# SensorsINI/v2e

Hardware: AMD Instinct MI355X
Metric: Mevents/s (EventEmulator.generate_events, 346x260, 10x slowdown) (higher is better)
Workload: dtype f64

## Files before the change

### v2e_amd/csrc/emu.hip

```cpp
#include "common.h"
#include "../../include/v2e_detmath.h"

#include <cstdarg>
#include <cstdlib>
#include <chrono>
#include <vector>

namespace {

constexpr int BLOCK = 256;
constexpr int WAVE = 64;
constexpr int RING = 64;
constexpr int SCAN_BLOCKS = 64;
constexpr int STAMP_LAUNCHES = 128;

constexpr uint32_t CNT_MASK = 0x00FFFFFFu;
constexpr uint32_t CNT_NEG = 1u << 24;
constexpr uint32_t CNT_SHOT_ON = 1u << 25;
constexpr uint32_t CNT_SHOT_OFF = 1u << 26;

struct FrameCtl {
    double t_prev, t_frame;
    double dt_over_tau;
    double shot_base;
// ... 579 lines not shown
                const unsigned long long row = ev0 + it_base + cidx;
                if (row < cap) ev[row] = make_float4(t, fx, fy, neg ? -1.0f : 1.0f);
                else dropped = true;
                ++fcount;
            }
        }
        carry += chunk_total;
    }
    const uint32_t son_tot = trow[2 * M], soff_tot = trow[2 * M + 1];
    if (a.do_shot) {
        const bool s_on = (cw & CNT_SHOT_ON) != 0, s_off = (cw & CNT_SHOT_OFF) != 0;
        const unsigned long long so = __ballot(s_on), sf = __ballot(s_off);
        if (so | sf) {
            const float tl = tg(n - 1);
            if (s_on) {
                const unsigned long long row = ev0 + carry + hrow[(size_t)(2 * M) * a.nwaves + w] + (uint32_t)__popcll(so & lt);
                if (row < cap) ev[row] = make_float4(tl, fx, fy, 1.0f);
                else dropped = true;
            }
            if (s_off) {
                const unsigned long long row = ev0 + carry + son_tot + hrow[(size_t)(2 * M + 1) * a.nwaves + w] + (uint32_t)__popcll(sf & lt);
                if (row < cap) ev[row] = make_float4(tl, fx, fy, -1.0f);
                else dropped = true;
            }
        }
    }
    if (valid) {
        const bool shot = a.do_shot && (cw & (CNT_SHOT_ON | CNT_SHOT_OFF));
        if (fcount > 0 || shot) {
            R b = ((R *)a.base)[sp];
            const float dp = (float)(neg ? 0 : fcount) * a.pos_thres[sp];
            const float dn = (float)(neg ? fcount : 0) * a.neg_thres[sp];
            b = b + (R)dp;
            b = b - (R)dn;
            if (shot) b = ((R *)a.lp)[sp];
            ((R *)a.base)[sp] = b;
        }
        if (use_refr && fcount > 0) a.ts_mem[sp] = tsm;
    }
    if (__ballot(dropped) != 0ull && lane == 0) atomicOr(&rec[clip].flags, V2E_FLAG_EVENTS_DROPPED);
    if (w == 0 && lane == 0) {
        rec[clip].n_signal = carry;
        rec[clip].n_events = carry + (a.do_shot ? son_tot + soff_tot : 0u);
        rec[clip].n_on = sum_on + (a.do_shot ? son_tot : 0u);
        rec[clip].n_off = sum_off + (a.do_shot ? soff_tot : 0u);
        rec[clip].ev_offset = ev0;
    }
}

__global__ __launch_bounds__(BLOCK) void k_permute(const float4 *__restrict__ in, float4 *__restrict__ out,
                                                   const int32_t *__restrict__ idx, unsigned long long row0,
                                                   unsigned long long n)
{
    const unsigned long long j = (unsigned long long)blockIdx.x * BLOCK + threadIdx.x;
    if (j < n) out[row0 + j] = in[row0 + (unsigned long long)idx[j]];
}

struct FrameScratch {
    v2e_frame_rec rec[2];
    FrameCtl ctl;
};

__global__ __launch_bounds__(256) void k_frame_rows_to_host(const float4 *__restrict__ ev, const v2e_frame_rec *__restrict__ rec,
                                                            float4 *__restrict__ out_rows, v2e_frame_rec *__restrict__ out_rec,
                                                            unsigned long long row0, unsigned long long max_rows,
                                                            v2e_frame_rec *__restrict__ rec_next)
{
    const v2e_frame_rec r = *rec;
    if (blockIdx.x == 0 && threadIdx.x == 0) {
        if (out_rec) *out_rec = r;
        if (rec_next) {
            v2e_frame_rec z;
            memset(&z, 0, sizeof(z));
            *rec_next = z;
        }
    }
    if (r.flags & (V2E_FLAG_EVENTS_DROPPED | V2E_FLAG_ITERS_CLAMPED)) return;
    const unsigned long long n = r.n_events < row0 + max_rows ? r.n_events : row0 + max_rows;
    for (unsigned long long i = row0 + (unsigned long long)blockIdx.x * 256 + threadIdx.x; i < n; i += (unsigned long long)gridDim.x * 256)
        out_rows[i] = ev[i];
}

#include "emu_chain.h"

}

namespace {
__global__ void k_zero_words(uint32_t *p, size_t n)
{
    const size_t i = (size_t)blockIdx.x * 256 + threadIdx.x;
    if (i < n) p[i] = 0u;
}
struct ZeroRanges { uint32_t *p[4]; unsigned long long n[4]; };
__global__ __launch_bounds__(256) void k_zero_ranges(ZeroRanges z)
{
    const unsigned long long i = (unsigned long long)blockIdx.x * 256 + threadIdx.x;
    unsigned long long base = 0;
#pragma unroll
    for (int r = 0; r < 4; ++r) {
        if (i >= base && i < base + z.n[r]) z.p[r][i - base] = 0u;
        base += z.n[r];
    }
}
}
static inline hipError_t zero_async(void *p, size_t bytes, hipStream_t s)
{
    const size_t n = (bytes + 3) / 4;
    if (n == 0) return hipSuccess;
    k_zero_words<<<(unsigned)((n + 255) / 256), 256, 0, s>>>((uint32_t *)p, n);
    return hipGetLastError();
}

struct RunScratch {
    FrameCtl *run_ctl = nullptr;
    uint32_t *run_fidx = nullptr;
    const void **run_frames = nullptr;
    unsigned long long **stamp_slot = nullptr;
    unsigned long long *run_off = nullptr;
    uint32_t *ch_gM = nullptr;
    unsigned *ch_bar = nullptr;
    uint2 *ch_rec = nullptr;
    uint32_t *ch_cnt = nullptr;
    uint32_t *ch_ruleM = nullptr;
    float *ch_tsold = nullptr;
    uint16_t *ch_wmax = nullptr;
    uint16_t *ch_wtot = nullptr;
    CFrame *ch_cf = nullptr;
    unsigned *ch_cdone = nullptr;
    uint32_t *ch_cT = nullptr, *ch_ckbase = nullptr, *ch_cperm = nullptr, *ch_cpre = nullptr;
    uint32_t *ch_cmask = nullptr;
    uint32_t *ch_cpre16 = nullptr;
    void free_chain()
    {
        auto drop = [](auto *&b) { hipFree((void *)b); b = nullptr; };
        drop(ch_gM); drop(ch_bar); drop(ch_rec); drop(ch_cnt); drop(ch_ruleM); drop(ch_tsold); drop(ch_wmax); drop(ch_wtot);
        drop(ch_cf); drop(ch_cdone); drop(ch_cT); drop(ch_ckbase); drop(ch_cperm); drop(ch_cpre); drop(ch_cmask); drop(ch_cpre16);
    }
    void free_all()
    {
        free_chain();
        auto drop = [](auto *&b) { hipFree((void *)b); b = nullptr; };
        drop(run_ctl); drop(run_fidx); drop(run_frames); drop(stamp_slot); drop(run_off);
    }
};

struct v2e_emu {
    int H, W, n_clips, max_iters, device;
    int npx, nwaves, nkeys_cap;
    long long npx_pad;
    void *lp = nullptr, *base = nullptr;
    float *ts_mem = nullptr, *pos_thres = nullptr, *neg_thres = nullptr, *noise_rate = nullptr;
    uint32_t *cnt = nullptr, *hist = nullptr, *tot = nullptr;
    void *pn_arr = nullptr;
    const float *pn_tape = nullptr;
    void *sc_hp = nullptr, *sc_prev = nullptr;
    const void *cs_sur = nullptr;
    void *csr_scratch = nullptr, *csr_lp = nullptr;
    std::vector<double> csr_ap, csr_ah;
    std::vector<int> csr_steps;
    double csr_thr = 0.0;
    int *csr_steps_dev = nullptr;
    unsigned long long *csr_slots = nullptr;
    int csr_slots_cap = 0;
    float *sc_tau = nullptr;
    uint32_t sc_first_frame = 0;
    double *dbg_lognew = nullptr, *dbg_cms = nullptr, *dbg_diff = nullptr;
// ... 1013 lines not shown
            V2E_HIP(hipDeviceSynchronize());
        }
        if (n_launch > h->ch_launch_cap) {
            h->sync_runs();
            for (RunScratch &q : h->sets) { hipFree(q.ch_gM); hipFree(q.ch_bar); q.ch_gM = nullptr; q.ch_bar = nullptr; }
            h->ch_launch_cap = n_launch;
            h->drop_graphs();
        }
        if (!r.ch_gM) {
            V2E_HIP(hipMalloc(&r.ch_gM, sizeof(uint32_t) * (size_t)h->ch_launch_cap * (K + 1) * h->n_clips * K));
            V2E_HIP(hipMalloc(&r.ch_bar, sizeof(unsigned) * (size_t)h->ch_launch_cap * 2 * K * h->n_clips));
            h->drop_graphs();
        }
    }
    return 0;
}

static bool chain_eligible(const v2e_emu *h, const v2e_emu_params *p, int dtype)
{
    if (h->max_iters > CHAIN_MAX_ITERS) return false;
    if (dtype == V2E_DT_F64 && p->log_input) return false;
    if (p->photoreceptor_noise) return false;
    if (h->sc_hp) return false;
    if (h->cs_sur) return false;
    return true;
}

enum class ChainMode {
    plain,
    captured,
    pipelined,
    profiled,
};
struct ChainMarks { std::vector<hipEvent_t> chain, rows; };

static int enqueue_run_chain(v2e_emu *h, const v2e_emu_params *p, const KArgs &a_in, int dtype, int n_frames, float *events,
                             uint64_t cap, v2e_frame_rec *recs, hipStream_t s, ChainMode mode, ChainMarks *marks = nullptr)
{
    const bool captured = mode == ChainMode::captured, pipelined = mode == ChainMode::pipelined;
    const RunScratch &r = h->cur();
    const size_t esz = dtype == V2E_DT_U8 ? 1 : (dtype == V2E_DT_F32 ? 4 : 8);
    const bool has_refr = p->refractory_period_s > 0;
    const int K = h->ch_K, E = h->ch_E, m = E / K, D = h->ch_D, NC = h->n_clips, nD = h->ch_nD;
    const bool fused_rec = h->ch_fused != 0;
    const std::vector<ChainLaunch> plan = chain_plan(n_frames, K, E, nD, has_refr, fused_rec);
    const int nL = (int)plan.size();
    const int nB = (n_frames + K - 1) / K;
    const int nEB = (n_frames + E - 1) / E;
    KArgs a = a_in;
    Sched sc;
    sc.h = h; sc.st[ST_MAIN] = s; sc.st[ST_AHEAD] = h->ahead; sc.st[ST_SIDE] = h->side; sc.st[ST_TAB] = h->tabs; sc.st[ST_SIDE2] = h->side2;
    if (mode == ChainMode::profiled)
        for (int q = 0; q < ST_COUNT; ++q) sc.st[q] = s;
    auto mark = [&](bool rows, hipStream_t stq) -> int {
        if (mode != ChainMode::profiled) return 0;
        hipEvent_t e;
        V2E_HIP(hipEventCreate(&e));
        (rows ? marks->rows : marks->chain).push_back(e);
        V2E_HIP(hipEventRecord(e, stq));
        return 0;
    };
    int gy = NC;
    if (has_refr && K > 1) gy = std::max(1, std::min(NC, h->ch_max_blocks / std::max(h->ngroups, 1)));
    dim3 grid(h->ngroups, gy);
    const int tab_stream = captured || pipelined ? ST_SIDE : ST_TAB;
    constexpr int NSET = 3;
    auto launch_emission = [&](int b, int ef0, int enE) -> int {
        CEmitArgs ea;
        memset(&ea, 0, sizeof(ea));
        ea.ctl = r.run_ctl; ea.recs = recs; ea.fidx_base = r.run_fidx;
        ea.f0 = ef0; ea.nE = enE; ea.D = D; ea.n_clips = NC; ea.slot0 = ef0 % D;
        ea.nwp = h->ch_nwp; ea.nwaves = chain_egroups(h); ea.E = E;
        ea.cnt = r.ch_cnt; ea.tsold = has_refr ? r.ch_tsold : nullptr; ea.ruleM = has_refr ? r.ch_ruleM : nullptr;
        const size_t set = (size_t)(b % NSET) * E * NC;
        ea.wmax = r.ch_wmax + set * h->ch_nwp; ea.wtot = r.ch_wtot + set * h->nkeys_cap * h->ch_nwp;
        ea.cf = r.ch_cf + set; ea.cT = r.ch_cT + set * h->nkeys_cap; ea.ckbase = r.ch_ckbase + set * h->nkeys_cap;
        ea.cperm = r.ch_cperm + set * h->max_iters * 8; ea.cpre = r.ch_cpre + set * h->nkeys_cap * h->ch_nwp;
        ea.cdone = r.ch_cdone + set;
        const bool pull = r.ch_cmask != nullptr;
        ea.cmask = pull ? r.ch_cmask + set * h->ch_nwp * h->nkeys_cap * 2 * GPX : nullptr;
        bool two = h->ch_nwp > 1024;
        if (const char *ev = getenv("V2E_AMD_PULL_TWO_LEVEL")) two = atoi(ev) != 0;
        ea.cpre16 = pull && two ? r.ch_cpre16 + set * h->nkeys_cap * (h->ch_nwp / 16) : nullptr;
        ea.wpf = std::max(4, std::min(two ? 128 : 64, h->npx / 2048));
        ea.p2 = two ? 16 : 64;
        while (ea.p2 < (two ? h->ch_nwp / 16 : ea.nwaves)) ea.p2 *= 2;
        ea.events = (float4 *)events; ea.cap = cap;
        ea.off_in = r.run_off + (size_t)b * NC;
        ea.off_out = r.run_off + (size_t)(b + 1) * NC;
        ea.ich = 4;
        ea.capw = GROUP_PX * ea.ich;
        ea.coff_in_cemit = captured || pipelined ? 1 : 0;
        ea.zpw_tot = CTOT_ZF;
        ea.zpw_emit = 1;
        const int REC_LDS = (ea.capw + WAVE) * 4 * (BLOCK / WAVE);
        const int egx = (chain_egroups(h) + BLOCK / WAVE - 1) / (BLOCK / WAVE);
        void *args[] = {(void *)&a, (void *)&ea};
        if (sc.wait(tab_stream, EV_FORK, b)) return V2E_EHIP;
        if (b >= NSET && !captured && sc.wait(tab_stream, EV_JOIN, b - NSET)) return V2E_EHIP;
        if (sc.kernel(tab_stream, (const void *)k_ctot, dim3(egx, NC, (ea.nE + CTOT_ZF - 1) / CTOT_ZF), dim3(BLOCK), 0, args)) return V2E_EHIP;
        if (h->ch_nwp <= 4096) {
            if (sc.kernel(tab_stream, (const void *)k_cframe1, dim3(1, NC, ea.nE), dim3(CFRAME_THREADS), 0, args)) return V2E_EHIP;
        } else if (sc.kernel(tab_stream, (const void *)k_cframe, dim3(std::min(h->nkeys_cap, CFRAME_ROWS), NC, ea.nE), dim3(CFRAME_THREADS), 0, args)) {
            return V2E_EHIP;
        }
        const int row_stream = pipelined ? ST_SIDE2 : captured ? ST_SIDE : ((b & 1) ? ST_SIDE2 : ST_SIDE);
        if (!ea.coff_in_cemit) {
            void *oargs[] = {(void *)&ea};
            if (sc.kernel(tab_stream, (const void *)k_coff, dim3(NC), dim3(WAVE), 0, oargs)) return V2E_EHIP;
        }
        if (sc.record(EV_TAB, b, tab_stream)) return V2E_EHIP;
        if (!captured && sc.wait(row_stream, EV_TAB, b)) return V2E_EHIP;
        if (mark(true, sc.st[row_stream])) return V2E_EHIP;
        if (pull) {
            if (sc.kernel(row_stream, ea.cpre16 ? (const void *)k_cpull<true> : (const void *)k_cpull<false>, dim3(8 * ea.wpf * ((ea.nE + 7) / 8), NC), dim3(BLOCK), (size_t)(2 * ea.p2 * 4), args)) return V2E_EHIP;
        } else if (sc.kernel(row_stream, (const void *)k_cemit, dim3(egx, NC, ea.nE), dim3(BLOCK), (size_t)REC_LDS, args)) return V2E_EHIP;
        if (mark(true, sc.st[row_stream])) return V2E_EHIP;
        return sc.record(EV_JOIN, b, row_stream);
    };
    const bool split0 = m > 1 && n_frames > K && !pipelined;
    const bool ahead_whole = pipelined && !fused_rec && n_frames <= D;
    auto launch_ahead = [&](int b) -> int {
        if (!ahead_whole && b >= nD && sc.wait(ST_AHEAD, EV_CHAIN, (b - nD + 1) * m)) return V2E_EHIP;
        const int b0 = ahead_whole ? 0 : b * E, b1 = ahead_whole ? n_frames : std::min((b + 1) * E, n_frames);
        const int cut = (b == 0 && split0) ? std::min(K, b1) : b1;
        for (int part = 0; part < 2; ++part) {
            const int f0 = part == 0 ? b0 : cut, f1 = part == 0 ? cut : b1;
            if (f1 <= f0) continue;
            AheadArgs aa;
            memset(&aa, 0, sizeof(aa));
            aa.frames_pp = r.run_frames; aa.frame_stride = (unsigned long long)NC * h->npx * esz;
            aa.ctl = r.run_ctl; aa.fidx_base = r.run_fidx;
            aa.f0 = f0; aa.nf = f1 - f0; aa.D = D; aa.n_clips = NC; aa.slot0 = f0 % D;
            aa.rec = r.ch_rec;
            {
                const int pairs = aa.nf / 2 + 1;
                const long long wg_xy = (long long)h->ngroups * NC;
                int zb = (int)std::min<long long>(pairs, std::max<long long>((4ll * h->n_cu + wg_xy - 1) / wg_xy, (pairs + 15) / 16));
                aa.ppt = (pairs + zb - 1) / zb;
            }
            void *args[] = {(void *)&a, (void *)&aa};
            if (sc.kernel(ST_AHEAD, (const void *)k_ahead<uint8_t>, dim3(h->ngroups, NC, (aa.nf / 2 + 1 + aa.ppt - 1) / aa.ppt), dim3(BLOCK), 0, args)) return V2E_EHIP;
            if (sc.record(EV_AHEAD, part == 0 ? b : nL, ST_AHEAD)) return V2E_EHIP;
        }
        return 0;
    };
    void *xb[2] = {h->base, has_refr ? h->ch_base2 : h->base}, *xl[2] = {h->lp, has_refr ? h->ch_lp2 : h->lp};
    float *xt[2] = {h->ts_mem, has_refr ? h->ch_ts2 : h->ts_mem};
    {
        void *const zp[4] = {recs, r.run_off, has_refr ? (void *)r.ch_gM : nullptr, has_refr ? (void *)r.ch_bar : nullptr};
        const size_t zb[4] = {sizeof(v2e_frame_rec) * (size_t)n_frames * NC, sizeof(unsigned long long) * NC,
                              sizeof(uint32_t) * (size_t)nL * (K + 1) * NC * K, sizeof(unsigned) * (size_t)nL * 2 * K * NC};
        if (sc.zero4(pipelined ? ST_AHEAD : ST_MAIN, zp, zb)) return V2E_EHIP;
    }
    if (!pipelined) {
        if (sc.record(EV_FORK, nL, ST_MAIN)) return V2E_EHIP;
        if (!captured && sc.wait(ST_SIDE, EV_FORK, nL)) return V2E_EHIP;
        if (!fused_rec && sc.wait(ST_AHEAD, EV_FORK, nL)) return V2E_EHIP;
        if (!captured && (sc.wait(ST_TAB, EV_FORK, nL) || sc.wait(ST_SIDE2, EV_FORK, nL))) return V2E_EHIP;
    }
    int last_ahead = -1;
    if (ahead_whole && launch_ahead(0)) return V2E_EHIP;
    if (pipelined && (sc.record(EV_FORK, nL, ST_AHEAD) || sc.wait(ST_MAIN, EV_FORK, nL))) return V2E_EHIP;
    for (int b = 0; b < std::min(nEB, 2) && !fused_rec && !ahead_whole; ++b) {
        if (launch_ahead(b)) return V2E_EHIP;
        last_ahead = b;
    }
    const int tail_f0 = (nB - 1) * K;
    const bool split_tail = has_refr && m > 1 && nB >= 2 && (nB - 1) % m != 0 && !pipelined;
    int last_emitted = -1;
    const bool allon = a_in.has_cutoff && a_in.do_leak && a_in.do_shot && a_in.has_refr;
    const void *kfn = chain_fn(p->f64_state != 0, dtype, fused_rec, allon);
    for (int L = 0; L < nL; ++L) {
        const ChainLaunch &pl = plan[L];
        const bool tail = pl.nf == 0;
        ChainArgs ca;
        memset(&ca, 0, sizeof(ca));
        ca.frames_pp = r.run_frames; ca.frame_stride = (unsigned long long)NC * h->npx * esz; ca.fidx_base = r.run_fidx;
        ca.ctl = r.run_ctl;
        ca.f0 = pl.f0; ca.nf = pl.nf; ca.pf0 = pl.pf0; ca.pnf = pl.pnf;
        ca.D = D; ca.n_clips = NC; ca.K = K; ca.ngroups = h->ngroups;
        ca.slot_f0 = pl.f0 % D; ca.slot_pf0 = pl.pf0 % D;
        ca.cnt = r.ch_cnt; ca.ruleM = r.ch_ruleM; ca.tsold = has_refr ? r.ch_tsold : nullptr;
        ca.rec = r.ch_rec;
        if (has_refr) {
            ca.gM_cur = r.ch_gM + (size_t)L * (K + 1) * NC * K;
            ca.gM_prev = r.ch_gM + (size_t)(L > 0 ? L - 1 : 0) * (K + 1) * NC * K;
            ca.bar_prev = r.ch_bar + (size_t)(L > 0 ? L - 1 : 0) * 2 * K * NC;
        }
        const int in = L % 2, out = tail ? 0 : (L + 1) % 2, pin = (L + 1) % 2;
        ca.base_in = xb[in]; ca.lp_in = xl[in]; ca.ts_in = xt[in];
        ca.base_fix = xb[in]; ca.lp_fix = xl[in]; ca.ts_fix = xt[in];
        ca.base_out = xb[out]; ca.lp_out = xl[out]; ca.ts_out = xt[out];
        ca.base_pin = xb[pin]; ca.lp_pin = xl[pin]; ca.ts_pin = xt[pin];
        if (has_refr && K > CHAIN_SUB && h->ch_ck) {
            const size_t plane = (size_t)(K / CHAIN_SUB - 1 + (K % CHAIN_SUB ? 1 : 0)) * NC * h->npx_pad;
            auto ck = [&](int par, char *&bp, char *&lpp, float *&tp) {
                char *q = (char *)h->ch_ck + (size_t)par * plane * 20;
// ... 529 lines not shown
```

### v2e_amd/csrc/emu_chain.h

```cpp
#pragma once

#ifndef V2E_CHAIN_LOCKSTEP
#define V2E_CHAIN_LOCKSTEP 0
#endif
#ifndef V2E_CHAIN_STAMPS
#define V2E_CHAIN_STAMPS 0
#endif

constexpr int CHAIN_K_MAX = 64;
constexpr int CFRAME_THREADS = 1024;
constexpr int CHAIN_SUB = 8;
constexpr int CHAIN_MAX_ITERS = 1024;

template <typename R> __device__ __forceinline__ R floor_div_pos(R a, R b)
{
    if (!(b > (R)0) || !(a >= (R)0)) return div_floor<R>(a, b);
    if (a < b) return (R)0;
    R q = floor(a / b);
    R r = fma(-q, b, a);
    if (r < (R)0) q -= (R)1;
    else if (r >= b) q += (R)1;
    return q;
}

__device__ __forceinline__ bool clip_barrier(unsigned *ctr, unsigned target, bool light = false)
{
    __shared__ int s_ok;
    asm volatile("s_waitcnt vmcnt(0)" ::: "memory");
    __syncthreads();
    if (threadIdx.x == 0) {
        if (!light) {
            __builtin_amdgcn_fence(__ATOMIC_RELEASE, "agent");
            asm volatile("s_waitcnt vmcnt(0)" ::: "memory");
        }
        __hip_atomic_fetch_add(ctr, 1u, __ATOMIC_RELAXED, __HIP_MEMORY_SCOPE_AGENT);
        unsigned spins = 0;
        int ok = 1;
        while (__hip_atomic_load(ctr, __ATOMIC_RELAXED, __HIP_MEMORY_SCOPE_AGENT) < target) {
            if (light) __builtin_amdgcn_s_sleep(1); else __builtin_amdgcn_s_sleep(4);
            if (++spins > 2000000u) { ok = 0; break; }
        }
        if (!light) __builtin_amdgcn_fence(__ATOMIC_ACQUIRE, "agent");
        s_ok = ok;
    }
    __syncthreads();
    return s_ok != 0;
}

struct FrameTab {
    float start, step, end;
    uint32_t refr_mask;
    __device__ __forceinline__ FrameTab(const FrameCtl *c, int lane)
        : start(c->ts_start[lane & 31]), step(c->ts_stepf[lane & 31]), end(c->ts_end), refr_mask(c->refr_mask) {}
};

__device__ __forceinline__ TsGen frame_tsgen(const KArgs &a, const FrameCtl *c, const FrameTab &ft, int n, bool &use_refr)
{
    if (n <= 32) {
        use_refr = a.has_refr && ((ft.refr_mask >> (n - 1)) & 1u);
        return TsGen(__uint_as_float(lane_value(__float_as_uint(ft.start), n - 1)), ft.end,
                     __uint_as_float(lane_value(__float_as_uint(ft.step), n - 1)), n);
    }
    const double t_prev = c->t_prev, t_frame = c->t_frame;
    use_refr = a.has_refr && a.refr > (t_frame - t_prev) / (double)n;
    FrameCtl cc;
    cc.t_prev = t_prev; cc.t_frame = t_frame;
    return TsGen(cc, n, nullptr);
}

typedef float v2e_f4 __attribute__((ext_vector_type(4)));
typedef unsigned int v2e_u4 __attribute__((ext_vector_type(4)));
typedef unsigned int v2e_u2 __attribute__((ext_vector_type(2)));

__device__ __forceinline__ double lane_value_d(double v, int idx)
{
    const unsigned long long u = (unsigned long long)__double_as_longlong(v);
    return __longlong_as_double((long long)(((unsigned long long)lane_value((uint32_t)(u >> 32), idx) << 32) | lane_value((uint32_t)u, idx)));
}
__device__ __forceinline__ void store_event_wt(float4 *ev_clip, unsigned long long row, float t, float x, float y, float pol)
{
    if (row < 0x7000000ull) {
        const __amdgpu_buffer_rsrc_t r = __builtin_amdgcn_make_buffer_rsrc((void *)ev_clip, 0, 0x7fffffff, 0x00020000);
        const v2e_f4 v = {t, x, y, pol};
// ... 583 lines not shown
    unsigned *cdone;
    int capw, ich;
    int zpw_tot, zpw_emit;
    int coff_in_cemit;
    uint32_t *cmask;
    int wpf, p2;
    uint32_t *cpre16;
};

#ifndef V2E_GPX
#define V2E_GPX 4
#endif
constexpr int GPX = V2E_GPX;
constexpr int GROUP_PX = GPX * WAVE;
constexpr int GROUP_SRC_BITS = GPX <= 4 ? 8 : (GPX <= 8 ? 9 : 10);

constexpr int CTOT_ZF = 2;

__global__ __launch_bounds__(BLOCK) void k_ctot(KArgs a, CEmitArgs ea)
{
    const int tid = threadIdx.x, lane = tid & (WAVE - 1), wave = tid / WAVE;
    const int clip = blockIdx.y;
    const int grp = blockIdx.x * (BLOCK / WAVE) + wave;
    if (grp >= ea.nwaves) return;
    const int p0 = grp * GROUP_PX + lane;
    const int zb = (int)blockIdx.z * CTOT_ZF;
    uint32_t cwq[CTOT_ZF][GPX], rMq[CTOT_ZF];
    int slotq[CTOT_ZF];
    {
        int sl = ea.slot0 + zb;
        if (sl >= ea.D) sl -= ea.D;
#pragma unroll
        for (int q = 0; q < CTOT_ZF; ++q) {
            slotq[q] = sl;
            rMq[q] = 0u;
#pragma unroll
            for (int j = 0; j < GPX; ++j) {
                cwq[q][j] = 0u;
                if (zb + q < ea.nE && p0 + j * WAVE < a.npx) cwq[q][j] = ea.cnt[((size_t)sl * ea.n_clips + clip) * a.npx_pad + p0 + j * WAVE];
            }
            if (zb + q < ea.nE && ea.ruleM) rMq[q] = ea.ruleM[(size_t)sl * ea.n_clips + clip];
            if (++sl == ea.D) sl = 0;
        }
    }
#pragma unroll
    for (int q = 0; q < CTOT_ZF; ++q) {
        const int z = zb + q;
        if (z >= ea.nE) break;
        const size_t zc = (size_t)z * ea.n_clips + clip;
        const uint32_t rM = (uint32_t)__builtin_amdgcn_readfirstlane((int)rMq[q]);
        int magv[GPX];
        bool neg[GPX];
        unsigned long long negb[GPX];
        int mmax = 0;
        uint32_t son = 0, soff = 0;
        unsigned long long sob[GPX], sfb[GPX];
#pragma unroll
        for (int j = 0; j < GPX; ++j) {
            const uint32_t cw = cwq[q][j];
            magv[j] = (int)(cw & CNT_MASK);
            neg[j] = (cw & CNT_NEG) != 0;
            negb[j] = __ballot(neg[j]);
            mmax = max(mmax, magv[j]);
            sob[j] = __ballot((cw & CNT_SHOT_ON) != 0);
            sfb[j] = __ballot((cw & CNT_SHOT_OFF) != 0);
            son += (uint32_t)__popcll(sob[j]);
            soff += (uint32_t)__popcll(sfb[j]);
        }
        const int wm = wave_max_i32(mmax);
        if (lane == 0) ea.wmax[zc * ea.nwp + grp] = (uint16_t)min(wm, 65535);
        uint16_t *trow = ea.wtot + (zc * a.nkeys_cap) * ea.nwp + grp;
        uint32_t *mrow = ea.cmask ? ea.cmask + ((zc * a.nkeys_cap + (lane >= 2 * GPX ? 1 : 0)) * ea.nwp + grp) * (2 * GPX) + (lane & (2 * GPX - 1)) : nullptr;
        auto put_masks = [&](const int key_on, const unsigned long long (&on_m)[GPX], const unsigned long long (&off_m)[GPX]) __attribute__((always_inline)) {
            uint32_t mw = 0u;
#pragma unroll
            for (int j = 0; j < GPX; ++j) {
                asm("v_writelane_b32 %0, %1, %2" : "+v"(mw) : "s"((uint32_t)on_m[j]), "n"(2 * j));
                asm("v_writelane_b32 %0, %1, %2" : "+v"(mw) : "s"((uint32_t)(on_m[j] >> 32)), "n"(2 * j + 1));
                asm("v_writelane_b32 %0, %1, %2" : "+v"(mw) : "s"((uint32_t)off_m[j]), "n"(2 * GPX + 2 * j));
                asm("v_writelane_b32 %0, %1, %2" : "+v"(mw) : "s"((uint32_t)(off_m[j] >> 32)), "n"(2 * GPX + 2 * j + 1));
            }
            if (lane < 4 * GPX) mrow[(size_t)key_on * ea.nwp * (2 * GPX)] = mw;
        };
        const int wmc = min(wm, a.max_iters);
        const int nkw = 2 + 2 * wmc;
        bool ruled = false;
        TsGen tg(0.f, 0.f, 0.f, 1);
        float tsm[GPX];
#pragma unroll
        for (int j = 0; j < GPX; ++j) tsm[j] = 0.f;
        if (rM != 0u) {
            const FrameCtl *c = ea.ctl + (size_t)(ea.f0 + z) * ea.n_clips + clip;
            const FrameTab ftb(c, lane);
            tg = frame_tsgen(a, c, ftb, (int)rM, ruled);
            if (ea.tsold) {
#pragma unroll
                for (int j = 0; j < GPX; ++j)
                    if (p0 + j * WAVE < a.npx) tsm[j] = ea.tsold[((size_t)slotq[q] * ea.n_clips + clip) * a.npx_pad + p0 + j * WAVE];
            }
        }
        for (int kb = 0; kb < nkw; kb += WAVE) {
            uint32_t mine = 0;
            const int i_lo = kb == 0 ? 0 : (kb - 2) / 2;
            const int i_hi = min((kb + WAVE - 2) / 2, wmc);
            for (int i = i_lo; i < i_hi; ++i) {
                uint32_t on = 0, off = 0;
                unsigned long long on_m[GPX], off_m[GPX];
                if (!ruled) {
#pragma unroll
                    for (int j = 0; j < GPX; ++j) {
                        const unsigned long long cb = __ballot(magv[j] > i);
                        on_m[j] = cb & ~negb[j];
                        off_m[j] = cb & negb[j];
                    }
                } else {
#pragma unroll
                    for (int j = 0; j < GPX; ++j) {
                        bool pass = magv[j] > i;
                        if (pass) {
                            const float t = tg(i);
                            const float pt = 1.0f * t - tsm[j];
                            pass = pt > a.refr_f;
                            if (pass) tsm[j] = t;
                        }
                        on_m[j] = __ballot(pass && !neg[j]);
                        off_m[j] = __ballot(pass && neg[j]);
                    }
                }
#pragma unroll
                for (int j = 0; j < GPX; ++j) {
                    on += (uint32_t)__popcll(on_m[j]);
                    off += (uint32_t)__popcll(off_m[j]);
                }
                if (mrow) put_masks(2 + 2 * i, on_m, off_m);
                const int kl = 2 + 2 * i - kb;
                if (lane == kl) mine = on;
                if (lane == kl + 1) mine = off;
            }
            if (kb == 0) {
                if (lane == 0) mine = son;
                if (lane == 1) mine = soff;
                if (mrow && (son | soff) != 0u) put_masks(0, sob, sfb);
            }
            if (kb + lane < nkw) trow[(size_t)(kb + lane) * ea.nwp] = (uint16_t)mine;
        }
    }
}

__device__ __forceinline__ void key_row16(const uint16_t *__restrict__ row_at, const uint16_t *__restrict__ wm_at, uint32_t k, uint32_t v[16])
{
    const uint4 t0 = *(const uint4 *)row_at, t1 = *(const uint4 *)(row_at + 8);
    const uint4 m0 = *(const uint4 *)wm_at, m1 = *(const uint4 *)(wm_at + 8);
    const uint32_t tw[8] = {t0.x, t0.y, t0.z, t0.w, t1.x, t1.y, t1.z, t1.w};
    const uint32_t mw[8] = {m0.x, m0.y, m0.z, m0.w, m1.x, m1.y, m1.z, m1.w};
#pragma unroll
    for (int j = 0; j < 16; ++j) {
        const uint32_t wmj = (mw[j >> 1] >> (16 * (j & 1))) & 0xFFFFu;
        v[j] = k < 2u + 2u * wmj ? ((tw[j >> 1] >> (16 * (j & 1))) & 0xFFFFu) : 0u;
    }
}

__global__ __launch_bounds__(CFRAME_THREADS) void k_cframe1(KArgs a, CEmitArgs ea)
{
    __shared__ int s_red[CFRAME_THREADS / WAVE];
    __shared__ uint32_t s_T[2 * CHAIN_MAX_ITERS + 2];
    constexpr int NW = CFRAME_THREADS / WAVE;
    const int tid = threadIdx.x, lane = tid & (WAVE - 1), wave = tid / WAVE;
    const int clip = blockIdx.y, z = blockIdx.z, fe = ea.f0 + z;
    const uint16_t *wm = ea.wmax + ((size_t)z * ea.n_clips + clip) * ea.nwp;
    int m = 0;
    for (int k = tid; k < ea.nwaves; k += CFRAME_THREADS) m = max(m, (int)wm[k]);
    m = wave_max_i32(m);
    if (lane == 0) s_red[wave] = m;
    __syncthreads();
    int M = 0;
#pragma unroll
    for (int q = 0; q < NW; ++q) M = max(M, s_red[q]);
    M = __builtin_amdgcn_readfirstlane(M);
    CFrame *cf = ea.cf + (size_t)z * ea.n_clips + clip;
    v2e_frame_rec *rec = ea.recs + (size_t)fe * ea.n_clips + clip;
    if (M > a.max_iters) {
        if (tid == 0) {
            cf->M = M; cf->n_events = 0u; cf->n_signal = 0u; cf->discarded = 1u;
            rec->max_events = M;
            atomicOr(&rec->flags, V2E_FLAG_ITERS_CLAMPED);
        }
        return;
    }
    const int nk = 2 + 2 * M;
    const uint16_t *tot = ea.wtot + ((size_t)z * ea.n_clips + clip) * a.nkeys_cap * ea.nwp;
    uint32_t *pre = ea.cpre + ((size_t)z * ea.n_clips + clip) * a.nkeys_cap * ea.nwp;
    for (int k = wave; k < nk; k += NW) {
        uint32_t carry = 0;
        for (int w0 = 0; w0 < ea.nwp; w0 += 16 * WAVE) {
            const int wi = w0 + lane * 16;
            uint32_t v[16];
#pragma unroll
            for (int j = 0; j < 16; ++j) v[j] = 0u;
            if (wi < ea.nwp) {
                key_row16(tot + (size_t)k * ea.nwp + wi, wm + wi, (uint32_t)k, v);
            }
            uint32_t lane_tot = 0;
#pragma unroll
            for (int j = 0; j < 16; ++j) lane_tot += v[j];
            uint32_t run = carry + wave_excl_scan_u32(lane_tot, lane);
            carry += wave_sum_u32(lane_tot);
            if (wi < ea.nwp) {
                uint32_t o[16];
#pragma unroll
                for (int j = 0; j < 16; ++j) { o[j] = run; run += v[j]; }
                uint4 *dst = (uint4 *)(pre + (size_t)k * ea.nwp + wi);
                if (ea.cpre16) ea.cpre16[(((size_t)z * ea.n_clips + clip) * a.nkeys_cap + k) * (ea.nwp / 16) + wi / 16] = o[0];
                dst[0] = make_uint4(o[0], o[1], o[2], o[3]);
                dst[1] = make_uint4(o[4], o[5], o[6], o[7]);
                dst[2] = make_uint4(o[8], o[9], o[10], o[11]);
                dst[3] = make_uint4(o[12], o[13], o[14], o[15]);
            }
// ... 317 lines not shown
        }
        uint32_t nrec = 0;
        bool alive = true;
        for (int i = i0; i < i1; ++i) {
            unsigned long long cb[GPX], cand_any = 0ull;
#pragma unroll
            for (int j = 0; j < GPX; ++j) { cb[j] = __ballot(mag[j] > i); cand_any |= cb[j]; }
            if (cand_any == 0ull) { alive = false; break; }
            uint32_t run_on = 0, run_off = 0;
#pragma unroll
            for (int j = 0; j < GPX; ++j) {
                if (!use_refr && cb[j] == 0ull) continue;
                const bool cand = mag[j] > i;
                bool pass = cand;
                unsigned long long bo, bf;
                if (use_refr) {
                    const float t = tg(i);
                    const float pt = (cand ? 1.0f : 0.0f) * t - tsm[j];
                    pass = pt > a.refr_f;
                    if (pass) tsm[j] = t;
                    bo = __ballot(pass && !neg[j]);
                    bf = __ballot(pass && neg[j]);
                } else {
                    bf = cb[j] & negb[j];
                    bo = cb[j] & ~negb[j];
                }
                {
                    const uint32_t rank = neg[j] ? run_off + (uint32_t)__popcll(bf & lt) : run_on + (uint32_t)__popcll(bo & lt);
                    const uint32_t pos = pass ? nrec + (uint32_t)__popcll((bo | bf) & lt) : (uint32_t)(ea.capw + lane);
                    rec_w[pos] = (uint32_t)(j * WAVE + lane) | ((uint32_t)(i - i0) << GROUP_SRC_BITS) | ((neg[j] ? 1u : 0u) << (GROUP_SRC_BITS + 5)) |
                                 (rank << (GROUP_SRC_BITS + 6));
                }
                nrec += (uint32_t)__popcll(bo | bf);
                run_on += (uint32_t)__popcll(bo);
                run_off += (uint32_t)__popcll(bf);
            }
        }
        for (uint32_t e0 = 0; e0 < nrec; e0 += WAVE) {
            const bool has = e0 + lane < nrec;
            const uint32_t r = has ? rec_w[e0 + lane] : 0u;
            const uint32_t src = r & ((1u << GROUP_SRC_BITS) - 1u);
            const int il = (int)((r >> GROUP_SRC_BITS) & 31u);
            const bool eneg = (r >> (GROUP_SRC_BITS + 5)) & 1u;
            const uint32_t rank = r >> (GROUP_SRC_BITS + 6);
            const int kl = 2 * il;
            const uint32_t it_base = (uint32_t)__shfl((int)kbase_k, kl);
            const uint32_t tot_on = (uint32_t)__shfl((int)T_k, kl);
            const uint32_t off = (uint32_t)__shfl((int)P_k, kl + (eneg ? 1 : 0));
            float ex, ey;
            pixel_xy((uint32_t)(grp * GROUP_PX) + src, ex, ey);
            uint32_t cidx = (eneg ? tot_on : 0u) + off + rank;
            if (shuf) {
                v2e_perm_t pm;
                pm.k[0] = (uint32_t)__shfl((int)pa.x, il); pm.k[1] = (uint32_t)__shfl((int)pa.y, il);
                pm.k[2] = (uint32_t)__shfl((int)pa.z, il); pm.k[3] = (uint32_t)__shfl((int)pa.w, il);
                pm.sh = (uint32_t)__shfl((int)pb.x, il); pm.a = (uint32_t)__shfl((int)pb.y, il);
                pm.amask = 0u; pm.n = (uint32_t)__shfl((int)pb.w, il);
                pm.rmask = (1u << pm.sh) - 1u;
                if (has) cidx = v2e_perm_apply(&pm, cidx);
            }
            if (has) store_row(it_base + cidx, tg(i0 + il), ex, ey, eneg ? -1.0f : 1.0f);
        }
        if (!alive) break;
    }
    if (a.do_shot && any_shot) {
        const uint32_t son_tot = cT[0];
        uint32_t son_off = n_signal + pre[0], soff_off = n_signal + son_tot + pre[(size_t)ea.nwp];
        const float tl = tg(n - 1);
#pragma unroll
        for (int j = 0; j < GPX; ++j) {
            if ((so[j] | sf[j]) != 0ull) {
                float fx, fy;
                pixel_xy((uint32_t)(p0 + j * WAVE), fx, fy);
                if (cw[j] & CNT_SHOT_ON) store_row(son_off + (uint32_t)__popcll(so[j] & lt), tl, fx, fy, 1.0f);
                if (cw[j] & CNT_SHOT_OFF) store_row(soff_off + (uint32_t)__popcll(sf[j] & lt), tl, fx, fy, -1.0f);
                son_off += (uint32_t)__popcll(so[j]);
                soff_off += (uint32_t)__popcll(sf[j]);
            }
        }
    }
}

static_assert(GPX == 4, "k_cpull selects a pixel of a 256-pixel group (v2e_nth_set_bit_256)");
template <bool TWO>
__global__ __launch_bounds__(BLOCK) void k_cpull(KArgs a, CEmitArgs ea)
{
    extern __shared__ uint32_t s_pre[];
    const int tid = threadIdx.x, lane = tid & (WAVE - 1);
    const int clip = blockIdx.y;
    const int blk = (int)blockIdx.x >> 3;
    const int z = (blk / ea.wpf) * 8 + ((int)blockIdx.x & 7), q = blk % ea.wpf;
    if (z >= ea.nE) return;
    const int fe = ea.f0 + z;
    const size_t zc = (size_t)z * ea.n_clips + clip;
    const CFrame *cf = ea.cf + zc;
    v2e_frame_rec *rec = ea.recs + (size_t)fe * ea.n_clips;
    const FrameCtl *c = ea.ctl + (size_t)fe * ea.n_clips + clip;
    const uint32_t *cT = ea.cT + zc * a.nkeys_cap, *ckb = ea.ckbase + zc * a.nkeys_cap;
    const uint32_t *pre = ea.cpre + zc * a.nkeys_cap * ea.nwp;
    const uint32_t *perm = ea.cperm + zc * a.max_iters * 8;
    const uint32_t *cmask = ea.cmask + zc * a.nkeys_cap * ea.nwp * (2 * GPX);
    const bool shuf = (a.rng_mode == V2E_RNG_PHILOX) && a.shuffle;
    const uint32_t off_lo = (uint32_t)ea.off_in[clip], off_hi = (uint32_t)(ea.off_in[clip] >> 32);
    const uint32_t nj = lane < z ? ea.cf[(size_t)lane * ea.n_clips + clip].n_events : 0u;
    const int M = __builtin_amdgcn_readfirstlane(cf->M);
    const uint32_t n_signal = (uint32_t)__builtin_amdgcn_readfirstlane((int)cf->n_signal);
    const uint32_t n_events = (uint32_t)__builtin_amdgcn_readfirstlane((int)cf->n_events);
    const uint32_t disc = (uint32_t)__builtin_amdgcn_readfirstlane((int)cf->discarded);
    const FrameTab ftb(c, lane);
    const unsigned long long ev0 = ((unsigned long long)off_hi << 32 | off_lo) + (unsigned long long)wave_sum_u32(nj & 0xFFFFFFu) +
                                   ((unsigned long long)wave_sum_u32(nj >> 24) << 24);
    if (q == 0 && tid == 0) {
        rec[clip].ev_offset = ev0;
        if (ea.coff_in_cemit && z == ea.nE - 1) ea.off_out[clip] = ev0 + n_events;
        if (ev0 + n_events > ea.cap || n_events > 0x7FFFFFFu) atomicOr(&rec[clip].flags, V2E_FLAG_EVENTS_DROPPED);
    }
    if (disc) return;
    const int n = M > 0 ? M : 1;
    bool use_refr;
    const TsGen tg = frame_tsgen(a, c, ftb, n, use_refr);
    const uint32_t ev0_lo = (uint32_t)__builtin_amdgcn_readfirstlane((int)(uint32_t)ev0), ev0_hi = (uint32_t)__builtin_amdgcn_readfirstlane((int)(uint32_t)(ev0 >> 32));
    const unsigned long long ev0u = ((unsigned long long)ev0_hi << 32) | ev0_lo;
    const unsigned long long room = ev0u < ea.cap ? ea.cap - ev0u : 0ull;
    unsigned long long frows64 = room < (unsigned long long)n_events ? room : (unsigned long long)n_events;
    if (frows64 > 0x7FFFFFFull) frows64 = 0x7FFFFFFull;
    const uint32_t frows = (uint32_t)frows64;
    const uint32_t per = ((frows + (uint32_t)ea.wpf - 1u) / (uint32_t)ea.wpf + (uint32_t)WAVE - 1u) & ~(uint32_t)(WAVE - 1);
    const uint32_t lo = (uint32_t)q * per, hi = min(lo + per, frows);
    if (lo >= hi) return;
    const __amdgpu_buffer_rsrc_t ev_rsrc = __builtin_amdgcn_make_buffer_rsrc((void *)(ea.events + (size_t)clip * ea.cap + ev0u), 0, (int)(frows * 16u), 0x00020000);
    const float rcpW = 1.0f / (float)a.W;
    const int P2 = ea.p2;
    bool staged = false;
    for (int i = 0; i <= M; ++i) {
        if (i == M && !a.do_shot) break;
        const int key0 = i < M ? 2 + 2 * i : 0;
        const uint32_t base = i < M ? ckb[key0] : n_signal;
        const uint32_t T_on = cT[key0], T_off = cT[key0 + 1];
        const uint32_t r_lo = max(lo, base), r_hi = min(hi, base + T_on + T_off);
        if (r_lo >= r_hi) continue;
        if (staged) __syncthreads();
        if (TWO) {
            const int nc16 = ea.nwp / 16;
            const uint32_t *pre16 = ea.cpre16 + (zc * a.nkeys_cap + key0) * nc16;
            for (int k = tid; k < 2 * P2; k += BLOCK) {
                const int kk = k & (P2 - 1);
                s_pre[k] = kk < nc16 ? pre16[(size_t)(k >= P2 ? nc16 : 0) + kk] : 0xFFFFFFFFu;
            }
        } else {
            for (int k = tid * 4; k < 2 * P2; k += BLOCK * 4) {
                const int kk = k & (P2 - 1);
                uint4 v = make_uint4(0xFFFFFFFFu, 0xFFFFFFFFu, 0xFFFFFFFFu, 0xFFFFFFFFu);
                if (kk < ea.nwp) v = *(const uint4 *)(pre + (size_t)(key0 + (k >= P2 ? 1 : 0)) * ea.nwp + kk);
                *(uint4 *)(s_pre + k) = v;
            }
        }
        __syncthreads();
        staged = true;
        v2e_perm_t pm;
        const bool sh_i = shuf && i < M;
        if (sh_i) {
            const uint32_t *pp = perm + (size_t)i * 8;
            pm.k[0] = pp[0]; pm.k[1] = pp[1]; pm.k[2] = pp[2]; pm.k[3] = pp[3];
            pm.sh = pp[4]; pm.a = pp[5]; pm.amask = 0u; pm.n = pp[7];
            pm.rmask = (1u << pm.sh) - 1u;
        }
        const float t = tg(i < M ? i : n - 1);
        for (uint32_t row = r_lo + (uint32_t)tid; row < r_hi; row += BLOCK) {
            const uint32_t jj = row - base;
            const uint32_t ci = sh_i ? v2e_perm_invert(&pm, jj) : jj;
            const bool eneg = ci >= T_on;
            const uint32_t cp = eneg ? ci - T_on : ci;
            const uint32_t *tab = s_pre + (eneg ? P2 : 0);
            uint32_t g = 0, gbase = 0;
            if (!TWO) {
                for (int st = P2 >> 1; st >= 1; st >>= 1) {
                    const uint32_t v = tab[g + st];
                    if (v <= cp) { g += st; gbase = v; }
                }
            } else {
                for (int st = P2 >> 1; st >= 1; st >>= 1) {
                    const uint32_t v = tab[g + st];
                    if (v <= cp) g += st;
                }
                const uint4 *lp = (const uint4 *)(pre + (size_t)(key0 + (eneg ? 1 : 0)) * ea.nwp + g * 16u);
                const uint4 q0 = lp[0], q1 = lp[1], q2 = lp[2], q3 = lp[3];
                const bool h8 = q2.x <= cp;
                const uint4 a0 = h8 ? q2 : q0, a1 = h8 ? q3 : q1;
                const bool h4 = a1.x <= cp;
                const uint4 b = h4 ? a1 : a0;
                const bool h2 = b.z <= cp;
                const uint32_t c0 = h2 ? b.z : b.x, c1 = h2 ? b.w : b.y;
                const bool h1 = c1 <= cp;
                gbase = h1 ? c1 : c0;
                g = g * 16u + (h8 ? 8u : 0u) + (h4 ? 4u : 0u) + (h2 ? 2u : 0u) + (h1 ? 1u : 0u);
            }
            const uint4 *mp = (const uint4 *)(cmask + ((size_t)(key0 + (eneg ? 1 : 0)) * ea.nwp + g) * (2 * GPX));
            const uint4 ma = mp[0], mb = mp[1];
            const uint32_t bit = v2e_nth_set_bit_256((unsigned long long)ma.x | ((unsigned long long)ma.y << 32), (unsigned long long)ma.z | ((unsigned long long)ma.w << 32),
                                                     (unsigned long long)mb.x | ((unsigned long long)mb.y << 32), (unsigned long long)mb.z | ((unsigned long long)mb.w << 32),
                                                     cp - gbase);
            const uint32_t p = g * (uint32_t)GROUP_PX + bit;
            uint32_t qy;
            if (a.npx < (1 << 24)) {
                qy = (uint32_t)((float)p * rcpW);
                if (qy * (uint32_t)a.W > p) --qy;
                else if ((qy + 1u) * (uint32_t)a.W <= p) ++qy;
            } else {
                qy = p / (uint32_t)a.W;
            }
            const v2e_f4 v = {t, (float)(p - qy * (uint32_t)a.W), (float)qy, eneg ? -1.0f : 1.0f};
            __builtin_amdgcn_raw_buffer_store_b128(v, ev_rsrc, (int)(row * 16u), 0, 19);
        }
    }
}
```

Measured before the change: 18330.

## Add bucketed prefix index for pull search, batch rows, and DPP mask packing

Result: faster. 19210, median of 6 (+4.8%).

```diff
diff --git a/v2e_amd/csrc/emu.hip b/v2e_amd/csrc/emu.hip
--- a/v2e_amd/csrc/emu.hip
+++ b/v2e_amd/csrc/emu.hip
@@ -685,6 +685,9 @@
 }
 
 #include "emu_chain.h"
+#ifndef V2E_PULL_PX_PER_WG
+#define V2E_PULL_PX_PER_WG 16384
+#endif
 
 }
 
@@ -1864,7 +1867,7 @@
         bool two = h->ch_nwp > 1024;
         if (const char *ev = getenv("V2E_AMD_PULL_TWO_LEVEL")) two = atoi(ev) != 0;
         ea.cpre16 = pull && two ? r.ch_cpre16 + set * h->nkeys_cap * (h->ch_nwp / 16) : nullptr;
-        ea.wpf = std::max(4, std::min(two ? 128 : 64, h->npx / 2048));
+        ea.wpf = std::max(4, std::min(two ? 128 : 64, h->npx / (two ? 2048 : V2E_PULL_PX_PER_WG)));
         ea.p2 = two ? 16 : 64;
         while (ea.p2 < (two ? h->ch_nwp / 16 : ea.nwaves)) ea.p2 *= 2;
         ea.events = (float4 *)events; ea.cap = cap;
@@ -1895,7 +1898,7 @@
         if (!captured && sc.wait(row_stream, EV_TAB, b)) return V2E_EHIP;
         if (mark(true, sc.st[row_stream])) return V2E_EHIP;
         if (pull) {
-            if (sc.kernel(row_stream, ea.cpre16 ? (const void *)k_cpull<true> : (const void *)k_cpull<false>, dim3(8 * ea.wpf * ((ea.nE + 7) / 8), NC), dim3(BLOCK), (size_t)(2 * ea.p2 * 4), args)) return V2E_EHIP;
+            if (sc.kernel(row_stream, ea.cpre16 ? (const void *)k_cpull<true> : (const void *)k_cpull<false>, dim3(8 * ea.wpf * ((ea.nE + 7) / 8), NC), dim3(BLOCK), (size_t)(2 * ea.p2 * (ea.cpre16 ? 4 : 6)), args)) return V2E_EHIP;
         } else if (sc.kernel(row_stream, (const void *)k_cemit, dim3(egx, NC, ea.nE), dim3(BLOCK), (size_t)REC_LDS, args)) return V2E_EHIP;
         if (mark(true, sc.st[row_stream])) return V2E_EHIP;
         return sc.record(EV_JOIN, b, row_stream);
diff --git a/v2e_amd/csrc/emu_chain.h b/v2e_amd/csrc/emu_chain.h
--- a/v2e_amd/csrc/emu_chain.h
+++ b/v2e_amd/csrc/emu_chain.h
@@ -1,4 +1,5 @@
 #pragma once
+#include "pull_index.h"
 
 #ifndef V2E_CHAIN_LOCKSTEP
 #define V2E_CHAIN_LOCKSTEP 0
@@ -748,6 +749,18 @@
             }
             if (lane < 4 * GPX) mrow[(size_t)key_on * ea.nwp * (2 * GPX)] = mw;
         };
+        static_assert(4 * GPX == 16, "k_ctot: the mask words of an iteration are one 16-lane DPP row");
+        uint32_t pmask = 0u;
+        if (mrow) {
+#pragma unroll
+            for (int j = 0; j < GPX; ++j) {
+                asm("v_writelane_b32 %0, %1, %2" : "+v"(pmask) : "s"((uint32_t)negb[j]), "n"(2 * j));
+                asm("v_writelane_b32 %0, %1, %2" : "+v"(pmask) : "s"((uint32_t)(negb[j] >> 32)), "n"(2 * j + 1));
+                asm("v_writelane_b32 %0, %1, %2" : "+v"(pmask) : "s"((uint32_t)negb[j]), "n"(2 * GPX + 2 * j));
+                asm("v_writelane_b32 %0, %1, %2" : "+v"(pmask) : "s"((uint32_t)(negb[j] >> 32)), "n"(2 * GPX + 2 * j + 1));
+            }
+            pmask = lane < 2 * GPX ? ~pmask : (lane < 4 * GPX ? pmask : 0u);
+        }
         const int wmc = min(wm, a.max_iters);
         const int nkw = 2 + 2 * wmc;
         bool ruled = false;
@@ -769,16 +782,12 @@
             uint32_t mine = 0;
             const int i_lo = kb == 0 ? 0 : (kb - 2) / 2;
             const int i_hi = min((kb + WAVE - 2) / 2, wmc);
+            uint32_t *mrow_i = mrow ? mrow + (size_t)(2 + 2 * i_lo) * ea.nwp * (2 * GPX) : nullptr;
             for (int i = i_lo; i < i_hi; ++i) {
-                uint32_t on = 0, off = 0;
-                unsigned long long on_m[GPX], off_m[GPX];
+                unsigned long long cb[GPX];
                 if (!ruled) {
 #pragma unroll
-                    for (int j = 0; j < GPX; ++j) {
-                        const unsigned long long cb = __ballot(magv[j] > i);
-                        on_m[j] = cb & ~negb[j];
-                        off_m[j] = cb & negb[j];
-                    }
+                    for (int j = 0; j < GPX; ++j) cb[j] = __ballot(magv[j] > i);
                 } else {
 #pragma unroll
                     for (int j = 0; j < GPX; ++j) {
@@ -789,16 +798,35 @@
                             pass = pt > a.refr_f;
                             if (pass) tsm[j] = t;
                         }
-                        on_m[j] = __ballot(pass && !neg[j]);
-                        off_m[j] = __ballot(pass && neg[j]);
+                        cb[j] = __ballot(pass);
                     }
                 }
-#pragma unroll
-                for (int j = 0; j < GPX; ++j) {
-                    on += (uint32_t)__popcll(on_m[j]);
-                    off += (uint32_t)__popcll(off_m[j]);
-                }
-                if (mrow) put_masks(2 + 2 * i, on_m, off_m);
+                uint32_t on, off;
+                if (mrow) {
+                    uint32_t mw = 0u;
+#pragma unroll
+                    for (int j = 0; j < GPX; ++j) {
+                        asm("v_writelane_b32 %0, %1, %2" : "+v"(mw) : "s"((uint32_t)cb[j]), "n"(2 * j));
+                        asm("v_writelane_b32 %0, %1, %2" : "+v"(mw) : "s"((uint32_t)(cb[j] >> 32)), "n"(2 * j + 1));
+                    }
+                    mw = (uint32_t)__builtin_amdgcn_update_dpp((int)mw, (int)mw, 0x118, 0xf, 0xc, false) & pmask;
+                    if (lane < 4 * GPX) *mrow_i = mw;
+                    mrow_i += (size_t)2 * ea.nwp * (2 * GPX);
+                    int c = __popc(mw);
+                    c += V2E_DPP(c, 0x111);
+                    c += V2E_DPP(c, 0x112);
+                    c += V2E_DPP(c, 0x114);
+                    on = (uint32_t)__builtin_amdgcn_readlane(c, 2 * GPX - 1);
+                    off = (uint32_t)__builtin_amdgcn_readlane(c, 4 * GPX - 1);
+                } else {
+                    on = 0u;
+                    off = 0u;
+#pragma unroll
+                    for (int j = 0; j < GPX; ++j) {
+                        on += (uint32_t)__popcll(cb[j] & ~negb[j]);
+                        off += (uint32_t)__popcll(cb[j] & negb[j]);
+                    }
+                }
                 const int kl = 2 + 2 * i - kb;
                 if (lane == kl) mine = on;
                 if (lane == kl + 1) mine = off;
@@ -1282,10 +1310,18 @@
 }
 
 static_assert(GPX == 4, "k_cpull selects a pixel of a 256-pixel group (v2e_nth_set_bit_256)");
+#ifndef V2E_PULL_ROWS
+#define V2E_PULL_ROWS 8
+#endif
+#ifndef V2E_PULL_ROWS_TWO
+#define V2E_PULL_ROWS_TWO 4
+#endif
 template <bool TWO>
 __global__ __launch_bounds__(BLOCK) void k_cpull(KArgs a, CEmitArgs ea)
 {
+    constexpr int PULL_ROWS = TWO ? V2E_PULL_ROWS_TWO : V2E_PULL_ROWS;
     extern __shared__ uint32_t s_pre[];
+    uint16_t *const s_idx = (uint16_t *)(s_pre + 2 * ea.p2);
     const int tid = threadIdx.x, lane = tid & (WAVE - 1);
     const int clip = blockIdx.y;
     const int blk = (int)blockIdx.x >> 3;
@@ -1339,6 +1375,7 @@
         const uint32_t T_on = cT[key0], T_off = cT[key0 + 1];
         const uint32_t r_lo = max(lo, base), r_hi = min(hi, base + T_on + T_off);
         if (r_lo >= r_hi) continue;
+        const uint32_t sh_on = pull_bucket_shift(T_on, (uint32_t)P2), sh_off = pull_bucket_shift(T_off, (uint32_t)P2);
         if (staged) __syncthreads();
         if (TWO) {
             const int nc16 = ea.nwp / 16;
@@ -1349,10 +1386,19 @@
             }
         } else {
             for (int k = tid * 4; k < 2 * P2; k += BLOCK * 4) {
-                const int kk = k & (P2 - 1);
+                const int kk = k & (P2 - 1), h = k >= P2 ? 1 : 0;
+                const uint32_t *src = pre + (size_t)(key0 + h) * ea.nwp;
                 uint4 v = make_uint4(0xFFFFFFFFu, 0xFFFFFFFFu, 0xFFFFFFFFu, 0xFFFFFFFFu);
-                if (kk < ea.nwp) v = *(const uint4 *)(pre + (size_t)(key0 + (k >= P2 ? 1 : 0)) * ea.nwp + kk);
+                uint32_t nx = 0xFFFFFFFFu;
+                if (kk < ea.nwp) v = *(const uint4 *)(src + kk);
+                if (kk + 4 < ea.nwp) nx = src[kk + 4];
                 *(uint4 *)(s_pre + k) = v;
+                const uint32_t T = h ? T_off : T_on, sh = h ? sh_off : sh_on;
+                uint16_t *ix = s_idx + h * P2;
+                pull_index_group(ix, (uint32_t)kk, v.x, v.y, T, sh);
+                pull_index_group(ix, (uint32_t)kk + 1u, v.y, v.z, T, sh);
+                pull_index_group(ix, (uint32_t)kk + 2u, v.z, v.w, T, sh);
+                pull_index_group(ix, (uint32_t)kk + 3u, v.w, nx, T, sh);
             }
         }
         __syncthreads();
@@ -1366,51 +1412,68 @@
             pm.rmask = (1u << pm.sh) - 1u;
         }
         const float t = tg(i < M ? i : n - 1);
-        for (uint32_t row = r_lo + (uint32_t)tid; row < r_hi; row += BLOCK) {
-            const uint32_t jj = row - base;
-            const uint32_t ci = sh_i ? v2e_perm_invert(&pm, jj) : jj;
-            const bool eneg = ci >= T_on;
-            const uint32_t cp = eneg ? ci - T_on : ci;
-            const uint32_t *tab = s_pre + (eneg ? P2 : 0);
-            uint32_t g = 0, gbase = 0;
-            if (!TWO) {
-                for (int st = P2 >> 1; st >= 1; st >>= 1) {
-                    const uint32_t v = tab[g + st];
-                    if (v <= cp) { g += st; gbase = v; }
-                }
-            } else {
-                for (int st = P2 >> 1; st >= 1; st >>= 1) {
-                    const uint32_t v = tab[g + st];
-                    if (v <= cp) g += st;
-                }
-                const uint4 *lp = (const uint4 *)(pre + (size_t)(key0 + (eneg ? 1 : 0)) * ea.nwp + g * 16u);
-                const uint4 q0 = lp[0], q1 = lp[1], q2 = lp[2], q3 = lp[3];
-                const bool h8 = q2.x <= cp;
-                const uint4 a0 = h8 ? q2 : q0, a1 = h8 ? q3 : q1;
-                const bool h4 = a1.x <= cp;
-                const uint4 b = h4 ? a1 : a0;
-                const bool h2 = b.z <= cp;
-                const uint32_t c0 = h2 ? b.z : b.x, c1 = h2 ? b.w : b.y;
-                const bool h1 = c1 <= cp;
-                gbase = h1 ? c1 : c0;
-                g = g * 16u + (h8 ? 8u : 0u) + (h4 ? 4u : 0u) + (h2 ? 2u : 0u) + (h1 ? 1u : 0u);
-            }
-            const uint4 *mp = (const uint4 *)(cmask + ((size_t)(key0 + (eneg ? 1 : 0)) * ea.nwp + g) * (2 * GPX));
-            const uint4 ma = mp[0], mb = mp[1];
-            const uint32_t bit = v2e_nth_set_bit_256((unsigned long long)ma.x | ((unsigned long long)ma.y << 32), (unsigned long long)ma.z | ((unsigned long long)ma.w << 32),
-                                                     (unsigned long long)mb.x | ((unsigned long long)mb.y << 32), (unsigned long long)mb.z | ((unsigned long long)mb.w << 32),
-                                                     cp - gbase);
-            const uint32_t p = g * (uint32_t)GROUP_PX + bit;
-            uint32_t qy;
-            if (a.npx < (1 << 24)) {
-                qy = (uint32_t)((float)p * rcpW);
-                if (qy * (uint32_t)a.W > p) --qy;
-                else if ((qy + 1u) * (uint32_t)a.W <= p) ++qy;
-            } else {
-                qy = p / (uint32_t)a.W;
-            }
-            const v2e_f4 v = {t, (float)(p - qy * (uint32_t)a.W), (float)qy, eneg ? -1.0f : 1.0f};
-            __builtin_amdgcn_raw_buffer_store_b128(v, ev_rsrc, (int)(row * 16u), 0, 19);
-        }
-    }
-}
+        for (uint32_t row0 = r_lo + (uint32_t)tid; row0 < r_hi; row0 += PULL_ROWS * BLOCK) {
+            uint32_t gv[PULL_ROWS], rv[PULL_ROWS];
+            bool nv[PULL_ROWS];
+            uint4 ma[PULL_ROWS], mb[PULL_ROWS];
+#pragma unroll
+            for (int u = 0; u < PULL_ROWS; ++u) {
+                const uint32_t row = row0 + (uint32_t)(u * BLOCK);
+                if (row >= r_hi) continue;
+                const uint32_t jj = row - base;
+                const uint32_t ci = sh_i ? v2e_perm_invert(&pm, jj) : jj;
+                const bool eneg = ci >= T_on;
+                const uint32_t cp = eneg ? ci - T_on : ci;
+                const uint32_t *tab = s_pre + (eneg ? P2 : 0);
+                uint32_t g = 0, gbase = 0;
+                if (!TWO) {
+                    g = pull_index_find(tab, s_idx + (eneg ? P2 : 0), eneg ? sh_off : sh_on, cp, &gbase);
+                } else {
+                    for (int st = P2 >> 1; st >= 1; st >>= 1) {
+                        const uint32_t v = tab[g + st];
+                        if (v <= cp) g += st;
+                    }
+                    const uint4 *lp = (const uint4 *)(pre + (size_t)(key0 + (eneg ? 1 : 0)) * ea.nwp + g * 16u);
+                    const uint4 q0 = lp[0], q1 = lp[1], q2 = lp[2], q3 = lp[3];
+                    const bool h8 = q2.x <= cp;
+                    const uint4 a0 = h8 ? q2 : q0, a1 = h8 ? q3 : q1;
+                    const bool h4 = a1.x <= cp;
+                    const uint4 b = h4 ? a1 : a0;
+                    const bool h2 = b.z <= cp;
+                    const uint32_t c0 = h2 ? b.z : b.x, c1 = h2 ? b.w : b.y;
+                    const bool h1 = c1 <= cp;
+                    gbase = h1 ? c1 : c0;
+                    g = g * 16u + (h8 ? 8u : 0u) + (h4 ? 4u : 0u) + (h2 ? 2u : 0u) + (h1 ? 1u : 0u);
+                }
+                const uint4 *mp = (const uint4 *)(cmask + ((size_t)(key0 + (eneg ? 1 : 0)) * ea.nwp + g) * (2 * GPX));
+                ma[u] = mp[0];
+                mb[u] = mp[1];
+                gv[u] = g;
+                rv[u] = cp - gbase;
+                nv[u] = eneg;
+            }
+#pragma unroll
+            for (int u = 0; u < PULL_ROWS; ++u) {
+                const uint32_t row = row0 + (uint32_t)(u * BLOCK);
+                if (row >= r_hi) continue;
+                const uint32_t bit = v2e_nth_set_bit_256((unsigned long long)ma[u].x | ((unsigned long long)ma[u].y << 32), (unsigned long long)ma[u].z | ((unsigned long long)ma[u].w << 32),
+                                                         (unsigned long long)mb[u].x | ((unsigned long long)mb[u].y << 32), (unsigned long long)mb[u].z | ((unsigned long long)mb[u].w << 32),
+                                                         rv[u]);
+                const uint32_t p = gv[u] * (uint32_t)GROUP_PX + bit;
+                uint32_t qy, qx;
+                if (a.npx < (1 << 24)) {
+                    qy = (uint32_t)((float)p * rcpW);
+                    int r = (int)(p - qy * (uint32_t)a.W);
+                    if (r < 0) { --qy; r += a.W; }
+                    else if (r >= a.W) { ++qy; r -= a.W; }
+                    qx = (uint32_t)r;
+                } else {
+                    qy = p / (uint32_t)a.W;
+                    qx = p - qy * (uint32_t)a.W;
+                }
+                const v2e_f4 v = {t, (float)qx, (float)qy, nv[u] ? -1.0f : 1.0f};
+                __builtin_amdgcn_raw_buffer_store_b128(v, ev_rsrc, (int)(row * 16u), 0, 19);
+            }
+        }
+    }
+}
diff --git a/v2e_amd/csrc/pull_index.h b/v2e_amd/csrc/pull_index.h
--- /dev/null
+++ b/v2e_amd/csrc/pull_index.h
@@ -0,0 +1,40 @@
+#pragma once
+#include <stdint.h>
+
+#if defined(__HIPCC__)
+#define V2E_PI_HD __host__ __device__ __forceinline__
+#else
+#define V2E_PI_HD static inline
+#endif
+
+V2E_PI_HD uint32_t pull_bucket_shift(uint32_t T, uint32_t nb)
+{
+    uint32_t s = 0;
+    if (T > 0u)
+        while (((T - 1u) >> s) + 2u > nb) ++s;
+    return s;
+}
+
+V2E_PI_HD void pull_index_group(uint16_t *idx, uint32_t g, uint32_t cur, uint32_t next, uint32_t T, uint32_t s)
+{
+    cur = cur < T ? cur : T;
+    next = next < T ? next : T;
+    if (cur >= next) return;
+    const uint32_t b0 = cur == 0u ? 0u : ((cur - 1u) >> s) + 1u;
+    uint32_t b1 = ((next - 1u) >> s) + 1u;
+    if (next == T) ++b1;
+    for (uint32_t b = b0; b < b1; ++b) idx[b] = (uint16_t)g;
+}
+
+V2E_PI_HD uint32_t pull_index_find(const uint32_t *tab, const uint16_t *idx, uint32_t s, uint32_t cp, uint32_t *gbase)
+{
+    const uint32_t b = cp >> s;
+    uint32_t lo = idx[b], hi = idx[b + 1u];
+    while (lo < hi) {
+        const uint32_t mid = (lo + hi + 1u) >> 1;
+        if (tab[mid] <= cp) lo = mid;
+        else hi = mid - 1u;
+    }
+    *gbase = tab[lo];
+    return lo;
+}
```
